# krejciadam/hammock

Measured on AMD Instinct MI355X. Metric: pairwise BLOSUM62 ShiftedScorer scores/sec (all-vs-all, thresholded neighbour list), higher is better.
Workload: dtype u8 (8-bit SWAR lanes, host-proven ranges with 16-bit / literal fallbacks; scores are int32-exact)

## Files before the change

hammock_amd/_native.py:

```python
from __future__ import annotations

import ctypes as C
import os

_HERE = os.path.dirname(os.path.abspath(__file__))
LIB_PATH = os.path.join(_HERE, "lib", "libhammock_hip.so")

HMK_OK = 0
HMK_ERR_BAD_ARG = 1
HMK_ERR_SHIFT_TOO_BIG = 2
HMK_ERR_DEVICE = 3
HMK_ERR_OOM = 4
HMK_ERR_REFERENCE_WOULD_CRASH = 5
HMK_ERR_CAPACITY = 6
HMK_ERR_NO_SEQUENCES = 7
HMK_EDGE_SHARDS = 64
HMK_MAX_LEN = 32
HMK_SURVEY_MAX_BINS = 1024
HMK_PROFILE_SYMBOLS = 21
HMK_PROFILE_MAX_WIDTH = 96
HMK_TARGET_MAX_LEN = 1 << 20
HMK_SCAN_ALL_WINDOWS = 1

SYMBOLS = [
    "hmk_abi_version", "hmk_last_kernel_ms", "hmk_create", "hmk_create_multi", "hmk_device_count", "hmk_destroy", "hmk_last_error", "hmk_set_sequences",
    "hmk_score_pairs_shifted", "hmk_score_with_shift", "hmk_score_pairs_local", "hmk_score_block_shifted", "hmk_score_block_local",
    "hmk_score_pairs_global", "hmk_score_block_global", "hmk_neighbors_global", "hmk_search_global", "hmk_align_pairs_global",
    "hmk_neighbors_shifted", "hmk_neighbors_local", "hmk_neighbors_shifted_dev", "hmk_compact_edges_dev", "hmk_pack_rows_dev", "hmk_unpack_rows_dev",
    "hmk_neighbors_last_plan", "hmk_neighbors_last_plan_shared", "hmk_neighbors_last_plan_tables", "hmk_search_shifted", "hmk_search_local", "hmk_search_best_shifted",
    "hmk_assign_shifted", "hmk_assign_local", "hmk_match_clusters_shifted", "hmk_match_clusters_local", "hmk_greedy_continue",
    "hmk_greedy_cluster", "hmk_greedy_from_edges", "hmk_greedy_from_edges_dev", "hmk_greedy_last_phases",
    "hmk_clinkage_cluster", "hmk_clinkage_from_edges", "hmk_set_java_hashset", "hmk_reserve",
    "hmk_cluster_pairs_shifted", "hmk_clinkage_merge", "hmk_clinkage_merge_from_edges",
    "hmk_cluster_linkage_shifted", "hmk_clinkage_split", "hmk_clinkage_split_from_edges",
    "hmk_components_shifted", "hmk_components_from_edges", "hmk_components_from_edges_dev",
    "hmk_cluster_align_shifted", "hmk_score_survey_shifted", "hmk_cluster_separation_shifted",
    "hmk_greedy_sweep", "hmk_greedy_sweep_from_edges", "hmk_greedy_sweep_from_edges_dev",
    "hmk_greedy_orders", "hmk_greedy_orders_from_edges",
    "hmk_representatives_shifted", "hmk_representatives_from_edges", "hmk_representatives_from_edges_dev",
    "hmk_density_shifted", "hmk_density_from_edges", "hmk_density_from_edges_dev",
    "hmk_cluster_profile", "hmk_set_targets", "hmk_scan_shifted",
]


# ... 177 lines not shown
    L.hmk_align_pairs_global.argtypes = [vp, p_u32, p_u32, u64, i32, i32, p_i32, p_u8, p_u64, p_u64]
    L.hmk_score_with_shift.argtypes = [vp, p_u32, p_u32, u64, i32, i32, p_i32, p_i32]
    L.hmk_score_block_shifted.argtypes = [vp, u32, u32, u32, u32, i32, i32, p_i32]
    L.hmk_score_block_local.argtypes = [vp, u32, u32, u32, u32, i32, i32, p_i32]
    L.hmk_score_block_global.argtypes = [vp, u32, u32, u32, u32, i32, i32, p_i32]
    L.hmk_neighbors_shifted.argtypes = [vp, i32, i32, i32, u32, u32, p_u64, u64, p_u64, C.POINTER(NeighborStats)]
    L.hmk_neighbors_local.argtypes = [vp, i32, i32, i32, u32, u32, p_u64, u64, p_u64, C.POINTER(NeighborStats)]
    L.hmk_neighbors_global.argtypes = [vp, i32, i32, i32, u32, u32, p_u64, u64, p_u64, C.POINTER(NeighborStats)]
    L.hmk_neighbors_shifted_dev.argtypes = [vp, i32, i32, i32, u32, u32, vp, u64, vp, vp]
    L.hmk_compact_edges_dev.argtypes = [vp, vp, u64, vp, vp, u64, vp, vp]
    L.hmk_pack_rows_dev.argtypes = [vp, vp, u64, vp, i32, vp, vp, u64, vp]
    L.hmk_unpack_rows_dev.argtypes = [vp, vp, vp, i32, vp, u64, vp]
    L.hmk_neighbors_last_plan.argtypes = [vp, C.POINTER(NeighborStats)]
    L.hmk_neighbors_last_plan_shared.argtypes = [vp, C.POINTER(C.c_uint32), C.POINTER(C.c_uint32)]
    L.hmk_neighbors_last_plan_tables.argtypes = [vp, C.POINTER(C.c_uint32), C.POINTER(C.c_uint64)]
    L.hmk_search_shifted.argtypes = [vp, u32, u32, u32, u32, i32, i32, i32, p_u64, u64, p_u64, C.POINTER(NeighborStats)]
    L.hmk_search_local.argtypes = [vp, u32, u32, u32, u32, i32, i32, i32, p_u64, u64, p_u64, C.POINTER(NeighborStats)]
    L.hmk_search_global.argtypes = [vp, u32, u32, u32, u32, i32, i32, i32, p_u64, u64, p_u64, C.POINTER(NeighborStats)]
    L.hmk_search_best_shifted.argtypes = [vp, u32, u32, u32, u32, i32, i32, i32, u32, p_u32, p_i32, p_u32, C.POINTER(NeighborStats)]
    L.hmk_assign_shifted.argtypes = [vp, u32, u32, u32, u32, p_u32, p_i32, u32, i32, i32, i32, u32, p_u32, p_i32, p_u32,
                                     C.POINTER(NeighborStats)]
    L.hmk_assign_local.argtypes = [vp, u32, u32, u32, u32, p_u32, p_i32, u32, i32, i32, i32, u32, p_u32, p_i32, p_u32,
                                   C.POINTER(NeighborStats)]
    L.hmk_match_clusters_shifted.argtypes = [vp, u32, u32, p_u32, u32, u32, u32, p_u32, p_i32, u32, i32, i32, i32, u32, p_u32, p_i32, p_u32,
                                             C.POINTER(NeighborStats)]
    L.hmk_match_clusters_local.argtypes = [vp, u32, u32, p_u32, u32, u32, u32, p_u32, p_i32, u32, i32, i32, i32, u32, p_u32, p_i32, p_u32,
                                           C.POINTER(NeighborStats)]
    L.hmk_greedy_continue.argtypes = [vp, u32, u32, u32, u32, p_u32, p_i32, u32, i32, i32, i32, p_i32, p_i32, C.POINTER(ContinueStats)]
    L.hmk_greedy_cluster.argtypes = [vp, i32, i32, i32, i32, p_i32, p_i32, p_i32, C.POINTER(GreedyStats)]
    L.hmk_greedy_from_edges_dev.argtypes = [vp, vp, u64, i32, i32, p_i32, p_i32, p_i32, C.POINTER(GreedyStats)]
# ... 54 lines not shown
```

hammock_amd/api.py:

```python
from __future__ import annotations

import ctypes as C

import numpy as np

from . import _native as N

AMINO_ACIDS = "ARNDCQEGHILKMFPSTWYVBZX*"
_NAME_TO_NUM = {c: i for i, c in enumerate(AMINO_ACIDS)}


class HammockException(Exception):
    """HammockException.java"""


class DataException(HammockException):
    """DataException.java -- e.g. "Shift too big" (ShiftedScorer.java:59-62)."""


class FileFormatException(HammockException):
    """FileFormatException.java"""


class DeviceError(HammockException):
# ... 544 lines not shown
            self._raise(st)

    def last_plan(self):
        stats = N.NeighborStats()
        st = N.lib.hmk_neighbors_last_plan(self._h, C.byref(stats))
        if st:
            self._raise(st)
        return stats

    def last_plan_shared(self):
        paired, shared = C.c_uint32(0), C.c_uint32(0)
        st = N.lib.hmk_neighbors_last_plan_shared(self._h, C.byref(paired), C.byref(shared))
        if st:
            self._raise(st)
        return int(paired.value), int(shared.value)

    def last_plan_tables(self):
        tiles, nbytes = C.c_uint32(0), C.c_uint64(0)
        st = N.lib.hmk_neighbors_last_plan_tables(self._h, C.byref(tiles), C.byref(nbytes))
        if st:
            self._raise(st)
        return int(tiles.value), int(nbytes.value)

    def greedy_cluster(self, max_shift, shift_penalty, threshold, max_clusters):
        cid = np.full(max(self.n, 1), -1, dtype=np.int32)
        order = np.full(max(self.n, 1), -1, dtype=np.int32)
        self.member_rank = np.zeros(max(self.n, 1), dtype=np.int32)
        stats = N.GreedyStats()
        st = N.lib.hmk_greedy_cluster(self._h, int(max_shift), int(shift_penalty), int(threshold), int(max_clusters),
                                      _ptr(cid, C.c_int32), _ptr(order, C.c_int32),
# ... 633 lines not shown
```

hammock_amd/csrc/hmk_api.cpp:

```cpp
#include "hmk_ctx.h"

using namespace hmk::impl;

extern "C" {

int hmk_abi_version(void) { return HMK_ABI_VERSION; }

double hmk_last_kernel_ms(const hmk_ctx *ctx) { return ctx ? ctx->last_kernel_ms : 0.0; }

const char *hmk_last_error(const hmk_ctx *ctx) { return ctx ? ctx->err.c_str() : g_last_error.c_str(); }

int hmk_create(const int32_t *matrix, int device, hmk_ctx **out) {
    if (!matrix || !out) return fail(nullptr, HMK_ERR_BAD_ARG, "hmk_create: null argument");
    *out = nullptr;
    hmk_ctx *ctx = new (std::nothrow) hmk_ctx();
    if (!ctx) return fail(nullptr, HMK_ERR_OOM, "out of memory");
    std::memcpy(ctx->M, matrix, sizeof(ctx->M));
    ctx->min_m = ctx->max_m = matrix[0];
    for (int e = 0; e < 576; e++) {
        ctx->min_m = std::min(ctx->min_m, matrix[e]);
        ctx->max_m = std::max(ctx->max_m, matrix[e]);
        if (matrix[e] != matrix[(e % 24) * 24 + e / 24]) ctx->symmetric = false;
        if (matrix[e] < -1000 || matrix[e] > 1000) {
            delete ctx;
// ... 253 lines not shown
    if (!ctx->plan.valid) return fail(ctx, HMK_ERR_BAD_ARG, "no neighbour pass has been planned yet");
    *stats = ctx->plan.stats;
    return HMK_OK;
}

int hmk_neighbors_last_plan_shared(hmk_ctx *ctx, uint32_t *paired_tiles, uint32_t *run_shared_tiles) {
    if (!ctx || !paired_tiles || !run_shared_tiles) return fail(ctx, HMK_ERR_BAD_ARG, "null argument");
    std::lock_guard<std::mutex> lock(ctx->mu);
    refresh_switches(ctx);
    if (!ctx->plan.valid) return fail(ctx, HMK_ERR_BAD_ARG, "no neighbour pass has been planned yet");
    *paired_tiles = ctx->plan.paired_tiles;
    *run_shared_tiles = ctx->plan.run_shared_tiles;
    return HMK_OK;
}

int hmk_neighbors_last_plan_tables(hmk_ctx *ctx, uint32_t *table_tiles, uint64_t *table_bytes) {
    if (!ctx || !table_tiles || !table_bytes) return fail(ctx, HMK_ERR_BAD_ARG, "null argument");
    std::lock_guard<std::mutex> lock(ctx->mu);
    refresh_switches(ctx);
    if (!ctx->plan.valid) return fail(ctx, HMK_ERR_BAD_ARG, "no neighbour pass has been planned yet");
    *table_tiles = ctx->plan.table_tiles;
    *table_bytes = ctx->plan.table_bytes;
    return HMK_OK;
}

int hmk_neighbors_shifted(hmk_ctx *ctx, int max_shift, int shift_penalty, int threshold, uint32_t part,
                          uint32_t n_parts, uint64_t *edges, uint64_t capacity, uint64_t *n_edges,
                          hmk_neighbor_stats *stats) {
    if (!ctx) return fail(nullptr, HMK_ERR_BAD_ARG, "null context");
    std::lock_guard<std::mutex> lock(ctx->mu);
// ... 290 lines not shown
```

hammock_amd/csrc/hmk_common.cpp:

```cpp
#include <atomic>

#include "hmk_ctx.h"
#include "hmk_grid.h"

namespace hmk {

static std::atomic<int> g_test_grid_cap{0};
void set_test_grid_cap(int cap) { g_test_grid_cap.store(cap < 1 ? 0 : cap, std::memory_order_relaxed); }
uint32_t capped_grid(const char *kernel, uint32_t wanted) {
    const int cap = g_test_grid_cap.load(std::memory_order_relaxed);
    if (cap < 1 || wanted <= (uint32_t)cap) return wanted;
    std::fprintf(stderr, "[hmk grid] %s %u -> %d\n", kernel, wanted, cap);
    return (uint32_t)cap;
}

namespace impl {

thread_local std::string g_last_error;

void Switches::read() {
    auto flag = [](const char *name) { return getenv(name) != nullptr; };
    auto num = [](const char *name, int dflt) { const char *v = getenv(name); return v ? atoi(v) : dflt; };
    *this = Switches();
    greedy_timing = flag("HMK_GREEDY_TIMING");
    no_band = flag("HMK_NO_BAND");
    no_rows_kernel = flag("HMK_NO_ROWS_KERNEL");
    key_sort = flag("HMK_NO_KEY_SORT") ? 0 : num("HMK_KEY_SORT_KEYS", 2) == 1 ? 1 : 2;
    no_row_shared = flag("HMK_NO_ROW_SHARED");
    key_row_pairs = getenv("HMK_KEY_ROW_PAIRS") ? (num("HMK_KEY_ROW_PAIRS", 0) != 0 ? 1 : 0) : -1;
    no_row_run_share = flag("HMK_NO_ROW_RUN_SHARE");
    no_tile_tables = flag("HMK_NO_TILE_TABLES");
    adj_8byte = flag("HMK_ADJ_8BYTE");
    local_literal = flag("HMK_LOCAL_LITERAL");
    local_signed = flag("HMK_LOCAL_SIGNED");
    local_no_pk = flag("HMK_LOCAL_NO_PK");
    multi_replicate = flag("HMK_MULTI_REPLICATE");
    multi_force_copies = flag("HMK_MULTI_FORCE_COPIES");
    if (const char *v = getenv("HMK_SECOND_LOOP")) second_loop = std::strcmp(v, "device") == 0 ? 1 : 2;
    phase1_threads = std::max(0, num("HMK_PHASE1_THREADS", 0));
    phase1_window = std::max(0, num("HMK_PHASE1_WINDOW", 0));
    if (const char *v = getenv("HMK_PHASE1_HOST_BAND")) {
        host_band_rows = std::max(0, atoi(v));
        if (const char *c = std::strchr(v, ',')) host_band_far_t = std::max(0, atoi(c + 1));
    }
    loop_chain = getenv("HMK_LOOP_CHAIN") ? (num("HMK_LOOP_CHAIN", 0) != 0 ? 1 : 0) : -1;
// ... 222 lines not shown
```

hammock_amd/csrc/hmk_ctx.h:

```cpp
#ifndef HMK_CTX_H
#define HMK_CTX_H
#include <hip/hip_runtime_api.h>

#include <algorithm>
#include <chrono>
#include <condition_variable>
#include <functional>
#include <future>
#include <memory>
#include <cstdio>
#include <cstdlib>
#include <cstring>
#include <map>
#include <mutex>
#include <numeric>
#include <string>
#include <tuple>
#include <thread>
#include <vector>

#include "hmk_internal.h"
#include "hmk_kernels.h"
#include "hmk_sizing.h"

// ... 68 lines not shown
    SB_SCAN_HITS, SB_SCAN_CNT,
    SB_SCAN_HASH, SB_SCAN_PAIRS, SB_SCAN_COV,
    SB_ORD_EDGES, SB_ORD_STATE, SB_ORD_POS,
    SB_ORD_IDS, SB_ORD_SUPPORT, SB_ORD_PARTNERS,
    SB_N
};

struct Switches {
    bool greedy_timing = false;
    bool no_band = false;
    bool no_rows_kernel = false;
    int key_sort = 2;
    bool no_row_shared = false;
    int key_row_pairs = -1;
    bool no_row_run_share = false;
    bool no_tile_tables = false;
    bool adj_8byte = false;
    bool local_literal = false;
    bool local_signed = false;
    bool local_no_pk = false;
    bool multi_replicate = false;
    bool multi_force_copies = false;
    int second_loop = 0;
    int phase1_threads = 0, phase1_window = 0;
    int host_band_rows = 0, host_band_far_t = 0;
    int loop_chain = -1;
    int loop_passes = 0;
    int precheck = 0;
    int late_buffers_delay_ms = 0;
    int csr_bucket_shift = 0;
// ... 16 lines not shown
struct Plan : PlanArrays {
    bool valid = false;
    int X = 0, p = 0, thr = 0;
    uint32_t part = 0, n_parts = 1;
    uint32_t band_rows = 0;
    int64_t band_req = 0;
    int lbmax = 12, lpad = 16;
    bool exact = false;
    bool rows_exact = false;
    bool no_rows_kernel = false;
    int key_sort = 2;
    bool row_shared = true;
    int key_row_pairs = -1;
    bool row_run_share = true;
    bool tile_tables = true;
    bool key_pairs = false;
    uint32_t paired_tiles = 0, run_shared_tiles = 0;
    uint32_t table_tiles = 0;
    uint64_t table_bytes = 0;
    uint32_t *d_keyrun = nullptr;
    uint32_t *d_keytab = nullptr;
    uint32_t cols_per_tile = 16384;
    uint8_t *d_mb = nullptr;
    std::vector<Group> groups;
    hmk_neighbor_stats stats{};
    uint64_t band_pairs = 0;
    uint32_t q0 = 0, q1 = 0, r0 = 0, r1 = 0;
};

struct PlanLocal : PlanArrays {
    bool valid = false;
    uint32_t part = 0, n_parts = 1;
// ... 304 lines not shown
```

hammock_amd/csrc/hmk_internal.h:

```cpp
#ifndef HMK_INTERNAL_H
#define HMK_INTERNAL_H

#include <stdint.h>

#include <functional>
#include <string>
#include <vector>

#include "../../include/hammock_hip.h"

namespace hmk {


enum { PATH_U8 = 0, PATH_U16 = 1, PATH_DIRECT = 2, PATH_ROWS = 3 };

struct TileClass {
    uint8_t la, lb;
    uint8_t nd;
    uint8_t case_b;
    uint8_t x;
    uint8_t path;
    uint8_t nw;
    uint8_t pad;
    int32_t g;
// ... 19 lines not shown
    uint64_t *edges;
    unsigned long long *counts;
    uint64_t cap_per_shard;
    uint32_t n_tiles;
    uint32_t lpad;
    uint32_t symmetric;
    uint32_t row_is_m;
    uint32_t perm_identity;
    uint32_t *deg;
    uint32_t deg_m_offset;
    const uint32_t *keyrun;
    const uint32_t *keytab;
};

constexpr int KEYTAB_DWORDS = 16;
constexpr int ROWS_KEY_PAIR_GROUPS = 2;
constexpr uint32_t ROWS_RUN_SHARED = 1u << 8;
constexpr uint32_t ROWS_TILE_TABLE = 1u << 9;
constexpr int ROWTAB_POSITIONS = 12;
constexpr int ROWTAB_DWORDS = ROWTAB_POSITIONS * 24 * 2;
constexpr int KEYGROUP_KEY_DWORDS = 2 * 24 * KEYTAB_DWORDS;
constexpr int KEYGROUP_DWORDS = KEYGROUP_KEY_DWORDS + ROWTAB_DWORDS;
constexpr bool rows_keyed(int x, int d, int cap, bool exact, int g) { return exact && d == 0 && (g == 1 || g == ROWS_KEY_PAIR_GROUPS) && x == 3 && cap == 12; }
constexpr int rows_key_pos(int x, int l, int q) { return l / 2 - 1 + q < x ? x : l / 2 - 1 + q; }

struct Nbr {
    uint32_t m;
    int32_t s;
    uint32_t id() const { return m; }
    int32_t score() const { return s; }
// ... 101 lines not shown
```

hammock_amd/csrc/hmk_plan.cpp:

```cpp
#include "hmk_ctx.h"

namespace hmk { namespace impl {

template <class T, class Cmp>
void parallel_stable_sort(std::vector<T> &v, Cmp before) {
    const size_t n = v.size();
    const unsigned hw = usable_cpus();
    size_t runs = 1;
    while (runs < 8 && runs < (hw ? hw : 1u) && n / (2 * runs) >= 32768) runs *= 2;
    if (runs == 1) { std::stable_sort(v.begin(), v.end(), before); return; }
    std::vector<size_t> cut(runs + 1);
    for (size_t r = 0; r <= runs; r++) cut[r] = n * r / runs;
    {
        std::vector<std::thread> pool;
        for (size_t r = 1; r < runs; r++) pool.emplace_back([&, r] { std::stable_sort(v.begin() + (long)cut[r], v.begin() + (long)cut[r + 1], before); });
        std::stable_sort(v.begin(), v.begin() + (long)cut[1], before);
        for (std::thread &th : pool) th.join();
    }
    std::vector<T> other(n);
    std::vector<T> *from = &v, *to = &other;
    for (size_t width = 1; width < runs; width *= 2) {
        std::vector<std::thread> pool;
        for (size_t r = 0; r < runs; r += 2 * width) {
            auto job = [&, r] {
// ... 247 lines not shown
        c.g = (int32_t)g;
        const int lpd = u16 ? 2 : 4, bits = u16 ? 16 : 8;
        const int ndw = (nd + lpd - 1) / lpd;
        c.nw = (uint8_t)ndw;
        for (int t = 0; t < nd; t++) c.cinit[t / lpd] |= (uint32_t)ci[t] << ((t % lpd) * bits);
    }
    *out = c;
}

int build_plan(hmk_ctx *ctx, int X, int p, int thr, uint32_t part, uint32_t n_parts, int64_t band_rows, bool key_sort_ok) {
    Plan &pl = ctx->plan;
    const int want_keys = key_sort_ok ? ctx->sw.key_sort : 0;
    if (pl.valid && pl.X == X && pl.p == p && pl.thr == thr && pl.part == part && pl.n_parts == n_parts &&
        (band_rows < 0 || pl.band_req == band_rows) && pl.no_rows_kernel == ctx->sw.no_rows_kernel && pl.key_sort == want_keys &&
        pl.row_shared == !ctx->sw.no_row_shared && pl.key_row_pairs == ctx->sw.key_row_pairs && pl.row_run_share == !ctx->sw.no_row_run_share &&
        pl.tile_tables == !ctx->sw.no_tile_tables)
        return HMK_OK;
    free_plan(pl);
    if (band_rows < 0) band_rows = 0;
    const int64_t band_req = band_rows;
    const bool plan_timing = ctx->sw.greedy_timing;
    const auto plan_t0 = std::chrono::steady_clock::now();
    auto plan_lap = [&](const char *what) {
        if (plan_timing)
            fprintf(stderr, "[hmk plan] %s at %.2f ms\n", what,
                    std::chrono::duration<double, std::milli>(std::chrono::steady_clock::now() - plan_t0).count());
    };
    const uint32_t n = ctx->n;
    if (n == 0) return fail(ctx, HMK_ERR_NO_SEQUENCES, "no sequences set (hmk_set_sequences)");
    if (X < 0) return fail(ctx, HMK_ERR_BAD_ARG, "max_shift must be >= 0");
    if (n_parts == 0 || part >= n_parts) return fail(ctx, HMK_ERR_BAD_ARG, "part must be < n_parts");
// ... 77 lines not shown
    if (use_rows && ctx->min_len == ctx->max_len) {
        TileClass t1;
        classify(ctx, ctx->min_len, ctx->min_len, X, p, thr, &t1);
        pl.rows_exact = (t1.path == PATH_U8 || (refine && all_rows_fit)) && rows_kernel_available(X, ctx->min_len, ctx->min_len, true);
    }
    if (!use_rows && ctx->min_len == 12 && ctx->max_len == 12 && X == 3) {
        TileClass t12;
        classify(ctx, 12, 12, X, p, thr, &t12);
        pl.exact = t12.path == PATH_U8 && t12.nw == 2;
    }
    pl.key_sort = want_keys;
    pl.row_shared = !ctx->sw.no_row_shared;
    pl.key_row_pairs = ctx->sw.key_row_pairs;
    pl.row_run_share = !ctx->sw.no_row_run_share;
    pl.tile_tables = !ctx->sw.no_tile_tables;
    std::vector<uint32_t> keyrun;
    const int L1 = ctx->min_len;
    const bool key_sorted = pl.key_sort > 0 && pl.rows_exact && !(refine && !all_rows_fit) &&
                            rows_keyed(X, 0, L1, true, rows_per_tile_rows(X, 0, L1, true) / 8) && n >= 2;
    if (key_sorted) {
        const int k0 = rows_key_pos(X, L1, 0), k1 = rows_key_pos(X, L1, 1);
        auto key_of = [&](uint32_t k) { return (uint32_t)ctx->res[ctx->off[k] + k0] * HMK_ALPHABET + ctx->res[ctx->off[k] + k1]; };
        const uint32_t b0 = band_end[L1], b1 = bucket[L1 + 1];
        std::vector<uint32_t> cnt(HMK_ALPHABET * HMK_ALPHABET + 1, 0u), sorted(perm.begin() + b0, perm.begin() + b1);
        for (uint32_t q = b0; q < b1; q++) cnt[key_of(perm[q]) + 1]++;
        for (int v = 0; v < HMK_ALPHABET * HMK_ALPHABET; v++) cnt[v + 1] += cnt[v];
        for (uint32_t q = b0; q < b1; q++) sorted[cnt[key_of(perm[q])]++] = perm[q];
        std::copy(sorted.begin(), sorted.end(), perm.begin() + b0);
        keyrun.resize(2 * (size_t)n);
        uint32_t r0 = 0, r01 = 0;
        for (uint32_t q = 0; q < n; q++) {
            const uint32_t k = perm[q], c0 = ctx->res[ctx->off[k] + k0], c1 = ctx->res[ctx->off[k] + k1];
            if (q > 0) {
                const uint32_t kp = perm[q - 1];
                const bool same0 = ctx->res[ctx->off[kp] + k0] == c0;
                r0 += same0 ? 0u : 1u;
                r01 += (pl.key_sort == 2 && same0 && ctx->res[ctx->off[kp] + k1] == c1) ? 0u : 1u;
            }
            keyrun[2 * (size_t)q] = r0 << 5 | c0;
            keyrun[2 * (size_t)q + 1] = r01 << 5 | c1;
        }
    }
    auto tiles_about = [&](uint64_t tile_rows, uint32_t cols) { return ((uint64_t)n / tile_rows / n_parts + 1) * ((uint64_t)n / (2 * cols) + 1); };
    auto cols_for = [&](uint64_t tile_rows) {
        uint32_t cols = 65536;
        while (cols > 16384 && tiles_about(tile_rows, cols) < 8 * 1792) cols /= 2;
        return cols;
    };
    constexpr uint64_t KEY_PAIR_MIN_TILES = 6 * 2048;
    const uint64_t paired_rows = key_sorted ? (uint64_t)rows_per_tile_rows(X, 0, L1, true, true) : 0;
    pl.key_pairs = paired_rows != 0 && (ctx->sw.key_row_pairs >= 0 ? ctx->sw.key_row_pairs == 1
                                                                   : tiles_about(paired_rows, cols_for(paired_rows)) >= KEY_PAIR_MIN_TILES);
    const uint64_t tile_rows = pl.key_pairs ? paired_rows : pl.rows_exact ? (uint64_t)rows_per_tile_rows(X, 0, ctx->min_len, true) : use_rows ? 16 : 6;
    pl.cols_per_tile = cols_for(tile_rows);
    while (pl.cols_per_tile > 4096 && ((uint64_t)n / tile_rows + 1) * ((uint64_t)n / (2 * pl.cols_per_tile) + 1) < 4096)
// ... 65 lines not shown
            }
            if (pl.key_pairs && pl.row_run_share && t.nrows == 8u * ROWS_KEY_PAIR_GROUPS && (t.row_shared & 3u) == 3u &&
                keys_at(t.row0 + 8) == keys_at(t.row0))
                t.row_shared |= ROWS_RUN_SHARED;
        }
        plan_lap("row-shared groups");
    }
    const bool tile_tables = key_sorted && pl.tile_tables && L1 == ROWTAB_POSITIONS;
    if (tile_tables)
        for (Tile &t : tiles) t.row_shared |= ROWS_TILE_TABLE;
    pl.table_tiles = tile_tables ? (uint32_t)tiles.size() : 0u;
    pl.table_bytes = tile_tables ? (uint64_t)((n + 7) / 8) * ROWTAB_DWORDS * 4 : 0u;
    pl.paired_tiles = pl.key_pairs ? (uint32_t)tiles.size() : 0u;
    pl.run_shared_tiles = 0;
    for (const Tile &t : tiles) pl.run_shared_tiles += (t.row_shared & ROWS_RUN_SHARED) ? 1u : 0u;

    st = upload_plan(ctx, pl, perm, (size_t)pl.lpad, 16, pl.exact ? 8 : 1, classes, tiles);
    if (!st) st = upload_biased_matrix(ctx, pl);
    if (st) return st;
    if (key_sorted) {
        if (classes.size() != 1) return fail(ctx, HMK_ERR_DEVICE, "key-sorted plan with more than one class");
        const uint32_t n_groups = (n + 7) / 8;
        const size_t tab_dwords = (size_t)n_groups * KEYGROUP_DWORDS;
        HIPCHK(ctx, hipMalloc((void **)&pl.d_keyrun, keyrun.size() * 4));
        HIPCHK(ctx, hipMemcpy(pl.d_keyrun, keyrun.data(), keyrun.size() * 4, hipMemcpyHostToDevice));
        HIPCHK(ctx, hipMalloc((void **)&pl.d_keytab, tab_dwords * 4));
        HIPCHK(ctx, launch_rows_keytab(pl.d_res_sorted, (uint32_t)pl.lpad, n, pl.d_mb, classes.at(0).case_b, X, L1, classes.at(0).cinit, pl.d_keytab,
                                       n_groups));
        if (tile_tables)
            HIPCHK(ctx, launch_rows_rowtab(pl.d_res_sorted, (uint32_t)pl.lpad, n, pl.d_mb, classes.at(0).case_b, X, L1, pl.row_shared, pl.d_keytab,
// ... 168 lines not shown
```

hammock_amd/csrc/k_neighbors_rows.h:

```cpp
#ifndef HMK_NEIGHBORS_ROWS_H
#define HMK_NEIGHBORS_ROWS_H
#include "hmk_device.h"

namespace hmk {

constexpr int ROWS_STAGE_CAPFORM = 320, ROWS_STAGE_EXACT = 640, ROWS_STAGE_SHORT = 1024;
constexpr int ROWS_INLOOP_MAXCELLS = 45;
constexpr int rows_cells(int x, int cap) { return cap * (2 * x + 1) - x * (x + 1); }
constexpr bool rows_inloop(int x, int cap) { return rows_cells(x, cap) > ROWS_INLOOP_MAXCELLS; }
constexpr bool rows_inloop_shape(int x, int d, int cap, bool exact) { return (exact && d > 0) || rows_inloop(x, cap); }
constexpr int rows_stage(int x, int d, int cap, bool exact) {
    return !exact ? ROWS_STAGE_CAPFORM : rows_inloop_shape(x, d, cap, exact) ? ROWS_STAGE_EXACT : ROWS_STAGE_SHORT;
}
constexpr int rows_groups(int x, int , int cap, bool exact) {
    return !exact ? 2 : rows_inloop(x, cap) ? 1 : 2;
}
constexpr bool rows_two_ended(int x, int d, int cap, bool exact, int g) { return exact && !rows_inloop_shape(x, d, cap, exact) && g == 2; }

template <typename T>
__device__ __forceinline__ T rows_table_read(uint32_t addr) {
    return *reinterpret_cast<const volatile HMK_LDS T *>((uintptr_t)addr);
}
constexpr int rows_waves(int nd, int cap, int lds_bytes, bool exact) {
    const int v = cap + 2 * nd + 36 + (exact ? 0 : 6);
// ... 188 lines not shown
            n += 2 * ((ops + 1) / 2) + ((role == 1 || role == 2) && halves == 2 ? 1 : 0);
        }
        return n;
    }
    static constexpr bool follower_covers(int skip) {
        if (!body_covers(skip, true)) return false;
        for (int u = 0; u < ND; u++)
            for (int j = plane_j0(u); j < plane_j1(u); j++) {
                int n = (ordinary(u, skip, true, j) ? 1 : 0) + (skipped(skip, j) ? 1 : 0);
                for (int h = 0; h < 2; h++)
                    if (run_carried(u, skip) && merged_half(u, skip, true, h) && merged_j(u, h) == j) n += (j + u - X == key_pos(h)) ? 1 : 2;
                if (n != 1) return false;
            }
        return true;
    }

    template <int GI, int SKIP = 0, bool RS = false>
    static __device__ __forceinline__ void accumulate(const uint32_t (&off)[CAP], const uint32_t (&toff)[NT], int lbs,
                                                      const uint32_t (&c0)[ND], const uint32_t (&c1)[ND], uint32_t (&W0)[ND], uint32_t (&W1)[ND]) {
        static_assert(SKIP == 0 || EXACT_LB, "key positions are skipped by the one-length forms only");
        static_assert(!RS || EXACT_LB, "row-shared groups: one-length forms only");
        const uint32_t (&ci)[ND] = c0;
        if constexpr (RS) {
            static_assert(body_covers(SKIP, true), "every cell of the overlap exactly once");
            u32x2 ml = {0u, 0u}, mh = {0u, 0u};
#pragma unroll
            for (int u = 0; u < ND; u++) {
                const bool hi = merged_half(u, SKIP, true, 1), lo = merged_half(u, SKIP, true, 0);
                if (hi) {
                    if (merged_reuse(u, SKIP, true)) mh = ml;
// ... 440 lines not shown

    const uint8_t *const res_sorted = P.res_sorted;
    const uint32_t lpad_s = P.lpad;

    constexpr bool INLOOP = rows_inloop_shape(X, D, CAP, EXACT_LB);
    constexpr bool DEFER = EXACT_LB && !INLOOP;
    const uint64_t ka64 = (uint64_t)(uintptr_t)__builtin_amdgcn_kernarg_segment_ptr();
    const uint32_t ka_lo = (uint32_t)ka64, ka_hi = (uint32_t)(ka64 >> 32);
    uint32_t acc[G];
#pragma unroll
    for (int g = 0; g < G; g++) acc[g] = 0;
    static_assert(!KEYED || (G <= 2 && 2 * ND <= KEYTAB_DWORDS), "key table entry; at most two row groups per tile");
    static_assert(!KEYED || (S::body_reads(3, false) == 58 && S::body_reads(1, false) == 65 && S::body_reads(0, false) == 72), "ordinary bodies");
    static_assert(!KEYED || (S::body_reads(3, true) == 54 && S::body_reads(1, true) == 60 && S::body_reads(0, true) == 66), "row-shared bodies (and the lead of a run-shared tile)");
    static_assert(!KEYED || (S::follower_reads(3) == 48 && S::follower_reads(1) == 53 && S::follower_reads(0) == 58), "followers of a run-shared tile");
    static_assert(!KEYED || (S::run_carried_planes(3) == 6 && S::run_carried_planes(1) == 7 && S::run_carried_planes(0) == 7), "dwords a lead hands over");
    static_assert(!KEYED || (S::run_body_adds(3, 2) == 62 && S::run_body_adds(1, 2) == 69 && S::run_body_adds(0, 2) == 75 && S::run_body_adds(3, 3) == 58 &&
                             S::run_body_adds(1, 3) == 64 && S::run_body_adds(0, 3) == 68), "sums of the lead and the follower");
    const uint32_t wave = __builtin_amdgcn_readfirstlane(tid >> 6);
    const uint32_t *kt_tile = nullptr, *kr_wave = nullptr;
    if (keyed) {
        kt_tile = P.keytab + (size_t)(T.row0 >> 3) * KEYGROUP_DWORDS;
        kr_wave = P.keyrun + 2 * (size_t)(T.col0 + wave * 64);
    }
    auto key_entry = [](const uint32_t *e, uint32_t (&k0)[ND], uint32_t (&k1)[ND]) {
#pragma unroll
        for (int u = 0; u + 1 < ND; u += 2) {
            const u32x4 a = rows_const_load<u32x4>(e + 2 * u);
            k0[u] = a.x; k1[u] = a.y; k0[u + 1] = a.z; k1[u + 1] = a.w;
        }
        if constexpr (ND & 1) {
            const u32x2 a = rows_const_load<u32x2>(e + 2 * (ND - 1));
            k0[ND - 1] = a.x; k1[ND - 1] = a.y;
        }
    };
    using No = std::false_type;
    using Yes = std::true_type;
    constexpr bool RUNS = KEYED && G >= 2;
    for (uint32_t bt = 0; bt < n_batches; bt++) {
        const uint32_t colrel = bt * 256 + tid;
        const uint32_t col = T.col0 + colrel;
        uint32_t words[S::LPADW], tw[S::TWN];
        S::load_words(res_sorted + (size_t)col * lpad_s, col < col_end, RUNS && interior, lbs, words, tw);
        int kmode = 0;
        u32x2 ra;
        if constexpr (KEYED) {
            const uint32_t wc0 = T.col0 + bt * 256 + wave * 64;
            if (keyed && wc0 < col_end) {
                const uint32_t last = min(63u, col_end - 1u - wc0);
                ra = rows_const_load<u32x2>(kr_wave);
                const u32x2 rb = rows_const_load<u32x2>(kr_wave + 2 * last);
                if (ra.x == rb.x) kmode = ra.y == rb.y ? 3 : 1;
            }
        }
        uint32_t off[CAP], toff[S::NT];
        S::offsets_of(words, tw, tab_addr, tab_addr, off, toff);
        const bool look = !DEFER || (bt & 3u) == 3u || bt + 1 == n_batches;
        uint32_t Pm[ND];

        if constexpr (RUNS) {
            static_assert(INLOOP && !DEFER && !TWO, "paired tiles: an in-loop shape");
            auto body = [&](auto gt, auto kt, auto rt, uint32_t (&W0)[ND], uint32_t (&W1)[ND]) __attribute__((always_inline)) {
                constexpr int g = decltype(gt)::value, KM = decltype(kt)::value;
                constexpr bool RUN = decltype(rt)::value;
                const uint32_t *const kt_group = kt_tile + (size_t)g * KEYGROUP_DWORDS;
                [[maybe_unused]] const bool row_shared = (rs_groups & (1u << g)) != 0;
                uint32_t ks0[ND], ks1[ND];
                if constexpr (KM == 3) {
                    uint32_t kb0[ND], kb1[ND];
                    key_entry(kt_group + (ra.x & 31u) * KEYTAB_DWORDS, ks0, ks1);
                    key_entry(kt_group + (24 + (ra.y & 31u)) * KEYTAB_DWORDS, kb0, kb1);
#pragma unroll
                    for (int u = 0; u < ND; u++) { ks0[u] += kb0[u]; ks1[u] += kb1[u]; }
                } else if constexpr (KM == 1) {
                    key_entry(kt_group + (ra.x & 31u) * KEYTAB_DWORDS, ks0, ks1);
#pragma unroll
                    for (int u = 0; u < ND; u++) asm volatile("" : "+s"(ks0[u]), "+s"(ks1[u]));
                }
                const uint32_t (&s0)[ND] = KM != 0 ? ks0 : ci;
                const uint32_t (&s1)[ND] = KM != 0 ? ks1 : ci;
                read_phase_begin(prio);
                if constexpr (RUN) S::template accumulate_run<g, KM, (g > 0)>(off, s0, s1, W0, W1, Pm);
                else if (row_shared) S::template accumulate<g, KM, true>(off, toff, lbs, s0, s1, W0, W1);
                else S::template accumulate<g, KM>(off, toff, lbs, s0, s1, W0, W1);
                read_phase_end(prio);
            };
            auto hits = [&](auto gt, auto ft, const uint32_t (&W0)[ND], const uint32_t (&W1)[ND]) __attribute__((always_inline)) {
                constexpr int g = decltype(gt)::value;
                constexpr bool FULL = decltype(ft)::value;
                uint32_t o0 = W0[0], o1 = W1[0];
#pragma unroll
                for (int u = 1; u < ND; u++) { o0 |= W0[u]; o1 |= W1[u]; }
                if (__ballot(((o0 | o1) & 0x80808080u) != 0) == 0) return;
                uint32_t rm0 = 0x80808080u, rm1 = 0x80808080u;
                if constexpr (!FULL) {
                    const uint32_t rows_here = T.nrows - 8 * g;
                    rm0 = rows_here >= 4 ? 0x80808080u : 0x80808080u & ((1u << (8 * rows_here)) - 1u);
                    rm1 = rows_here >= 8 ? 0x80808080u : rows_here <= 4 ? 0u : 0x80808080u & ((1u << (8 * (rows_here - 4))) - 1u);
                }
                uint32_t hm = ((o0 & rm0) >> 4) | (o1 & rm1);
// ... 144 lines not shown
                                else stage[cnt + mbcnt64(mask)] = rec;
                            }
                            hm &= hm - 1u;
                        }
                        if constexpr (TWO && g == 1) cnt_hi += (uint32_t)__popcll(mask);
                        else cnt += (uint32_t)__popcll(mask);
                    }
                    if (!full) break;
                    flush_stage_rows<X, D, CAP, EXACT_LB, G, MODE>(stage, cnt, cnt_hi, tab_addr, ka_lo, ka_hi);
                    cnt = 0;
                    cnt_hi = 0;
                }
            };
            rows_for_each_group(std::make_integer_sequence<int, G>{}, one_group);
        }
        kr_wave += 2 * 256;
    }
    flush_stage_rows<X, D, CAP, EXACT_LB, G, MODE>(stage, cnt, cnt_hi, tab_addr, ka_lo, ka_hi);
}

template <int X, int D, int CAP, bool EXACT_LB, int G, int MODE>
__global__ void __launch_bounds__(256, rows_waves(2 * X + D + 1, CAP, rows_lds_bytes(X, D, CAP, EXACT_LB, G), EXACT_LB))
k_neighbors_rows(const NeighborParams P, const uint32_t tile_base) {
    __shared__ __attribute__((aligned(16))) uint8_t smem[rows_lds_bytes(X, D, CAP, EXACT_LB, G)];
    rows_tile<X, D, CAP, EXACT_LB, G, MODE>(P, tile_base, smem);
}

constexpr int ROWS_LENS_MAXLA = 20;
constexpr int rows_lens_first(int capb) { return capb <= 12 ? 6 : capb <= 16 ? 13 : 17; }
constexpr bool rows_lens_has(int x, int d, int capb, int lb) { return lb >= rows_lens_first(capb) && lb <= capb && lb >= 2 * x && lb + d <= ROWS_LENS_MAXLA; }
constexpr int rows_lens_lds(int x, int d, int capb) {
// ... 35 lines not shown
```

include/hammock_hip.h:

```cpp
#ifndef HAMMOCK_HIP_H
#define HAMMOCK_HIP_H

#include <stdint.h>

#ifdef __cplusplus
extern "C" {
#endif

#define HMK_ABI_VERSION 4
#define HMK_ALPHABET 24
#define HMK_MAX_LEN 32
#define HMK_MAX_SEQUENCES (1u << 24)
#define HMK_EDGE_SHARDS 64

typedef enum {
    HMK_OK = 0,
    HMK_ERR_BAD_ARG = 1,
    HMK_ERR_SHIFT_TOO_BIG = 2,
    HMK_ERR_DEVICE = 3,
    HMK_ERR_OOM = 4,
    HMK_ERR_REFERENCE_WOULD_CRASH = 5,
    HMK_ERR_CAPACITY = 6,
    HMK_ERR_NO_SEQUENCES = 7
} hmk_status;
// ... 58 lines not shown
int hmk_neighbors_global(hmk_ctx *ctx, int gap_open, int gap_extend, int threshold, uint32_t part,
                         uint32_t n_parts, uint64_t *edges, uint64_t capacity, uint64_t *n_edges,
                         hmk_neighbor_stats *stats);

int hmk_neighbors_shifted_dev(hmk_ctx *ctx, int max_shift, int shift_penalty, int threshold,
                              uint32_t part, uint32_t n_parts, void *d_edges, uint64_t capacity,
                              void *d_counts, void *stream);
int hmk_compact_edges_dev(hmk_ctx *ctx, const void *d_edges, uint64_t capacity, const void *d_counts,
                          void *d_out, uint64_t out_capacity, void *d_total, void *stream);
int hmk_pack_rows_dev(hmk_ctx *ctx, const void *d_edges, uint64_t capacity, const void *d_counts, int threshold,
                      void *d_row_start, void *d_adj, uint64_t adj_capacity, void *stream);
int hmk_unpack_rows_dev(hmk_ctx *ctx, const void *d_row_start, const void *d_adj, int threshold, void *d_edges_out,
                        uint64_t out_capacity, void *stream);
int hmk_neighbors_last_plan(hmk_ctx *ctx, hmk_neighbor_stats *stats);
int hmk_neighbors_last_plan_shared(hmk_ctx *ctx, uint32_t *paired_tiles, uint32_t *run_shared_tiles);
int hmk_neighbors_last_plan_tables(hmk_ctx *ctx, uint32_t *table_tiles, uint64_t *table_bytes);


int hmk_search_shifted(hmk_ctx *ctx, uint32_t q0, uint32_t q1, uint32_t r0, uint32_t r1,
                       int max_shift, int shift_penalty, int threshold,
                       uint64_t *edges, uint64_t capacity, uint64_t *n_edges, hmk_neighbor_stats *stats);
int hmk_search_local(hmk_ctx *ctx, uint32_t q0, uint32_t q1, uint32_t r0, uint32_t r1,
                     int gap_open, int gap_extend, int threshold,
                     uint64_t *edges, uint64_t capacity, uint64_t *n_edges, hmk_neighbor_stats *stats);
int hmk_search_global(hmk_ctx *ctx, uint32_t q0, uint32_t q1, uint32_t r0, uint32_t r1,
                      int gap_open, int gap_extend, int threshold,
                      uint64_t *edges, uint64_t capacity, uint64_t *n_edges, hmk_neighbor_stats *stats);
int hmk_search_best_shifted(hmk_ctx *ctx, uint32_t q0, uint32_t q1, uint32_t r0, uint32_t r1,
                            int max_shift, int shift_penalty, int threshold, uint32_t k,
                            uint32_t *hit_index, int32_t *hit_score, uint32_t *n_hits,
// ... 442 lines not shown
```

Baseline: 2664 billion.

## Keep key-skipping fast path for windows straddling one key-run boundary

Widens the per-column key-run record to four dwords so it also stores where the column's two-key run starts. A 64-column wave window that crosses exactly one boundary between key runs now takes the both-keys-skipped path. Lanes past the boundary then add a scalar-loaded correction, the difference between two key-table entries, to their accumulators. Before, such windows fell back to the slower single-key or no-key path. The cost is twice the key-run memory and extra scalar loads and adds on split windows. Plan statistics and an env switch to disable the feature are also added.

```diff
diff --git a/hammock_amd/_native.py b/hammock_amd/_native.py
--- a/hammock_amd/_native.py
+++ b/hammock_amd/_native.py
@@ -27,7 +27,7 @@
     "hmk_score_pairs_shifted", "hmk_score_with_shift", "hmk_score_pairs_local", "hmk_score_block_shifted", "hmk_score_block_local",
     "hmk_score_pairs_global", "hmk_score_block_global", "hmk_neighbors_global", "hmk_search_global", "hmk_align_pairs_global",
     "hmk_neighbors_shifted", "hmk_neighbors_local", "hmk_neighbors_shifted_dev", "hmk_compact_edges_dev", "hmk_pack_rows_dev", "hmk_unpack_rows_dev",
-    "hmk_neighbors_last_plan", "hmk_neighbors_last_plan_shared", "hmk_neighbors_last_plan_tables", "hmk_search_shifted", "hmk_search_local", "hmk_search_best_shifted",
+    "hmk_neighbors_last_plan", "hmk_neighbors_last_plan_shared", "hmk_neighbors_last_plan_split", "hmk_neighbors_last_plan_tables", "hmk_search_shifted", "hmk_search_local", "hmk_search_best_shifted",
     "hmk_assign_shifted", "hmk_assign_local", "hmk_match_clusters_shifted", "hmk_match_clusters_local", "hmk_greedy_continue",
     "hmk_greedy_cluster", "hmk_greedy_from_edges", "hmk_greedy_from_edges_dev", "hmk_greedy_last_phases",
     "hmk_clinkage_cluster", "hmk_clinkage_from_edges", "hmk_set_java_hashset", "hmk_reserve",
@@ -235,6 +235,7 @@
     L.hmk_neighbors_last_plan.argtypes = [vp, C.POINTER(NeighborStats)]
     L.hmk_neighbors_last_plan_shared.argtypes = [vp, C.POINTER(C.c_uint32), C.POINTER(C.c_uint32)]
     L.hmk_neighbors_last_plan_tables.argtypes = [vp, C.POINTER(C.c_uint32), C.POINTER(C.c_uint64)]
+    L.hmk_neighbors_last_plan_split.argtypes = [vp, C.POINTER(C.c_uint64), C.POINTER(C.c_uint64), C.POINTER(C.c_uint64)]
     L.hmk_search_shifted.argtypes = [vp, u32, u32, u32, u32, i32, i32, i32, p_u64, u64, p_u64, C.POINTER(NeighborStats)]
     L.hmk_search_local.argtypes = [vp, u32, u32, u32, u32, i32, i32, i32, p_u64, u64, p_u64, C.POINTER(NeighborStats)]
     L.hmk_search_global.argtypes = [vp, u32, u32, u32, u32, i32, i32, i32, p_u64, u64, p_u64, C.POINTER(NeighborStats)]
diff --git a/hammock_amd/api.py b/hammock_amd/api.py
--- a/hammock_amd/api.py
+++ b/hammock_amd/api.py
@@ -582,6 +582,13 @@
         if st:
             self._raise(st)
         return int(paired.value), int(shared.value)
+
+    def last_plan_split(self):
+        w, s, k = C.c_uint64(0), C.c_uint64(0), C.c_uint64(0)
+        st = N.lib.hmk_neighbors_last_plan_split(self._h, C.byref(w), C.byref(s), C.byref(k))
+        if st:
+            self._raise(st)
+        return int(w.value), int(s.value), int(k.value)
 
     def last_plan_tables(self):
         tiles, nbytes = C.c_uint32(0), C.c_uint64(0)
diff --git a/hammock_amd/csrc/hmk_api.cpp b/hammock_amd/csrc/hmk_api.cpp
--- a/hammock_amd/csrc/hmk_api.cpp
+++ b/hammock_amd/csrc/hmk_api.cpp
@@ -291,6 +291,17 @@
     return HMK_OK;
 }
 
+int hmk_neighbors_last_plan_split(hmk_ctx *ctx, uint64_t *windows, uint64_t *straddling_windows, uint64_t *split_windows) {
+    if (!ctx || !windows || !straddling_windows || !split_windows) return fail(ctx, HMK_ERR_BAD_ARG, "null argument");
+    std::lock_guard<std::mutex> lock(ctx->mu);
+    refresh_switches(ctx);
+    if (!ctx->plan.valid) return fail(ctx, HMK_ERR_BAD_ARG, "no neighbour pass has been planned yet");
+    *windows = ctx->plan.key_windows;
+    *straddling_windows = ctx->plan.straddling_windows;
+    *split_windows = ctx->plan.split_windows;
+    return HMK_OK;
+}
+
 int hmk_neighbors_last_plan_tables(hmk_ctx *ctx, uint32_t *table_tiles, uint64_t *table_bytes) {
     if (!ctx || !table_tiles || !table_bytes) return fail(ctx, HMK_ERR_BAD_ARG, "null argument");
     std::lock_guard<std::mutex> lock(ctx->mu);
diff --git a/hammock_amd/csrc/hmk_common.cpp b/hammock_amd/csrc/hmk_common.cpp
--- a/hammock_amd/csrc/hmk_common.cpp
+++ b/hammock_amd/csrc/hmk_common.cpp
@@ -29,6 +29,7 @@
     no_row_shared = flag("HMK_NO_ROW_SHARED");
     key_row_pairs = getenv("HMK_KEY_ROW_PAIRS") ? (num("HMK_KEY_ROW_PAIRS", 0) != 0 ? 1 : 0) : -1;
     no_row_run_share = flag("HMK_NO_ROW_RUN_SHARE");
+    no_key_split = flag("HMK_NO_KEY_SPLIT");
     no_tile_tables = flag("HMK_NO_TILE_TABLES");
     adj_8byte = flag("HMK_ADJ_8BYTE");
     local_literal = flag("HMK_LOCAL_LITERAL");
diff --git a/hammock_amd/csrc/hmk_ctx.h b/hammock_amd/csrc/hmk_ctx.h
--- a/hammock_amd/csrc/hmk_ctx.h
+++ b/hammock_amd/csrc/hmk_ctx.h
@@ -106,6 +106,7 @@
     bool no_row_shared = false;
     int key_row_pairs = -1;
     bool no_row_run_share = false;
+    bool no_key_split = false;
     bool no_tile_tables = false;
     bool adj_8byte = false;
     bool local_literal = false;
@@ -152,8 +153,10 @@
     int key_row_pairs = -1;
     bool row_run_share = true;
     bool tile_tables = true;
+    bool key_split = true;
     bool key_pairs = false;
     uint32_t paired_tiles = 0, run_shared_tiles = 0;
+    uint64_t key_windows = 0, straddling_windows = 0, split_windows = 0;
     uint32_t table_tiles = 0;
     uint64_t table_bytes = 0;
     uint32_t *d_keyrun = nullptr;
diff --git a/hammock_amd/csrc/hmk_internal.h b/hammock_amd/csrc/hmk_internal.h
--- a/hammock_amd/csrc/hmk_internal.h
+++ b/hammock_amd/csrc/hmk_internal.h
@@ -57,6 +57,7 @@
 };
 
 constexpr int KEYTAB_DWORDS = 16;
+constexpr int KEYRUN_DWORDS = 4;
 constexpr int ROWS_KEY_PAIR_GROUPS = 2;
 constexpr uint32_t ROWS_RUN_SHARED = 1u << 8;
 constexpr uint32_t ROWS_TILE_TABLE = 1u << 9;
diff --git a/hammock_amd/csrc/hmk_plan.cpp b/hammock_amd/csrc/hmk_plan.cpp
--- a/hammock_amd/csrc/hmk_plan.cpp
+++ b/hammock_amd/csrc/hmk_plan.cpp
@@ -285,7 +285,7 @@
     if (pl.valid && pl.X == X && pl.p == p && pl.thr == thr && pl.part == part && pl.n_parts == n_parts &&
         (band_rows < 0 || pl.band_req == band_rows) && pl.no_rows_kernel == ctx->sw.no_rows_kernel && pl.key_sort == want_keys &&
         pl.row_shared == !ctx->sw.no_row_shared && pl.key_row_pairs == ctx->sw.key_row_pairs && pl.row_run_share == !ctx->sw.no_row_run_share &&
-        pl.tile_tables == !ctx->sw.no_tile_tables)
+        pl.tile_tables == !ctx->sw.no_tile_tables && pl.key_split == !ctx->sw.no_key_split)
         return HMK_OK;
     free_plan(pl);
     if (band_rows < 0) band_rows = 0;
@@ -393,6 +393,7 @@
     pl.key_row_pairs = ctx->sw.key_row_pairs;
     pl.row_run_share = !ctx->sw.no_row_run_share;
     pl.tile_tables = !ctx->sw.no_tile_tables;
+    pl.key_split = !ctx->sw.no_key_split;
     std::vector<uint32_t> keyrun;
     const int L1 = ctx->min_len;
     const bool key_sorted = pl.key_sort > 0 && pl.rows_exact && !(refine && !all_rows_fit) &&
@@ -406,18 +407,21 @@
         for (int v = 0; v < HMK_ALPHABET * HMK_ALPHABET; v++) cnt[v + 1] += cnt[v];
         for (uint32_t q = b0; q < b1; q++) sorted[cnt[key_of(perm[q])]++] = perm[q];
         std::copy(sorted.begin(), sorted.end(), perm.begin() + b0);
-        keyrun.resize(2 * (size_t)n);
-        uint32_t r0 = 0, r01 = 0;
+        keyrun.assign((size_t)KEYRUN_DWORDS * n, 0u);
+        uint32_t r0 = 0, r01 = 0, start = 0;
         for (uint32_t q = 0; q < n; q++) {
             const uint32_t k = perm[q], c0 = ctx->res[ctx->off[k] + k0], c1 = ctx->res[ctx->off[k] + k1];
             if (q > 0) {
                 const uint32_t kp = perm[q - 1];
                 const bool same0 = ctx->res[ctx->off[kp] + k0] == c0;
                 r0 += same0 ? 0u : 1u;
-                r01 += (pl.key_sort == 2 && same0 && ctx->res[ctx->off[kp] + k1] == c1) ? 0u : 1u;
+                const bool same01 = pl.key_sort == 2 && same0 && ctx->res[ctx->off[kp] + k1] == c1;
+                r01 += same01 ? 0u : 1u;
+                if (!same01) start = q;
             }
-            keyrun[2 * (size_t)q] = r0 << 5 | c0;
-            keyrun[2 * (size_t)q + 1] = r01 << 5 | c1;
+            keyrun[(size_t)KEYRUN_DWORDS * q] = r0 << 5 | c0;
+            keyrun[(size_t)KEYRUN_DWORDS * q + 1] = r01 << 5 | c1;
+            keyrun[(size_t)KEYRUN_DWORDS * q + 2] = start;
         }
     }
     auto tiles_about = [&](uint64_t tile_rows, uint32_t cols) { return ((uint64_t)n / tile_rows / n_parts + 1) * ((uint64_t)n / (2 * cols) + 1); };
@@ -513,6 +517,22 @@
     pl.paired_tiles = pl.key_pairs ? (uint32_t)tiles.size() : 0u;
     pl.run_shared_tiles = 0;
     for (const Tile &t : tiles) pl.run_shared_tiles += (t.row_shared & ROWS_RUN_SHARED) ? 1u : 0u;
+    pl.key_windows = pl.straddling_windows = pl.split_windows = 0;
+    const bool splits = key_sorted && pl.key_pairs && pl.key_sort == 2 && pl.key_split;
+    if (key_sorted && !splits)
+        for (uint32_t q = 0; q < n; q++) keyrun[(size_t)KEYRUN_DWORDS * q + 2] = 0u;
+    if (key_sorted && pl.key_pairs) {
+        for (const Tile &t : tiles)
+            for (uint32_t w0 = t.col0; w0 < t.col0 + t.ncols; w0 += 64) {
+                const uint32_t last = std::min(63u, t.col0 + t.ncols - 1u - w0);
+                const uint32_t *a = &keyrun[(size_t)KEYRUN_DWORDS * w0], *b = &keyrun[(size_t)KEYRUN_DWORDS * (w0 + last)];
+                pl.key_windows++;
+                if (a[1] == b[1]) continue;
+                pl.straddling_windows++;
+                if ((b[1] >> 5) - (a[1] >> 5) == 1u && b[2] - w0 - 1u < last) pl.split_windows++;
+            }
+        plan_lap("split windows");
+    }
 
     st = upload_plan(ctx, pl, perm, (size_t)pl.lpad, 16, pl.exact ? 8 : 1, classes, tiles);
     if (!st) st = upload_biased_matrix(ctx, pl);
diff --git a/hammock_amd/csrc/k_neighbors_rows.h b/hammock_amd/csrc/k_neighbors_rows.h
--- a/hammock_amd/csrc/k_neighbors_rows.h
+++ b/hammock_amd/csrc/k_neighbors_rows.h
@@ -226,6 +226,16 @@
             }
         return true;
     }
+    static constexpr int split_starts(int side, int which) { return (which == 0 ? 1 : 0) + (side == 1 ? (which == 1 ? 1 : -1) : 0); }
+    static constexpr bool split_covers(bool rs) {
+        for (int side = 0; side < 2; side++)
+            if (split_starts(side, side) != 1 || split_starts(side, 1 - side) != 0) return false;
+        for (int u = 0; u < ND; u++)
+            for (int j = plane_j0(u); j < plane_j1(u); j++)
+                if (skipped(3, j) != (j == key_pos(0) || j == key_pos(1))) return false;
+        return rs ? follower_covers(3) : body_covers(3, false);
+    }
+    static constexpr int split_adds() { return 2 * ND; }
 
     template <int GI, int SKIP = 0, bool RS = false>
     static __device__ __forceinline__ void accumulate(const uint32_t (&off)[CAP], const uint32_t (&toff)[NT], int lbs,
@@ -696,14 +706,15 @@
     static_assert(!KEYED || (S::body_reads(3, false) == 58 && S::body_reads(1, false) == 65 && S::body_reads(0, false) == 72), "ordinary bodies");
     static_assert(!KEYED || (S::body_reads(3, true) == 54 && S::body_reads(1, true) == 60 && S::body_reads(0, true) == 66), "row-shared bodies (and the lead of a run-shared tile)");
     static_assert(!KEYED || (S::follower_reads(3) == 48 && S::follower_reads(1) == 53 && S::follower_reads(0) == 58), "followers of a run-shared tile");
-    static_assert(!KEYED || (S::run_carried_planes(3) == 6 && S::run_carried_planes(1) == 7 && S::run_carried_planes(0) == 7), "dwords a lead hands over");
+    static_assert(!KEYED || (S::body_reads(3, false) == 58 && S::body_reads(3, true) == 54 && S::follower_reads(3) == 48), "a split window reads what a both-keys window reads");
+    static_assert(!KEYED || (S::run_carried_planes(3) == 6&& S::run_carried_planes(1) == 7 && S::run_carried_planes(0) == 7), "dwords a lead hands over");
     static_assert(!KEYED || (S::run_body_adds(3, 2) == 62 && S::run_body_adds(1, 2) == 69 && S::run_body_adds(0, 2) == 75 && S::run_body_adds(3, 3) == 58 &&
                              S::run_body_adds(1, 3) == 64 && S::run_body_adds(0, 3) == 68), "sums of the lead and the follower");
     const uint32_t wave = __builtin_amdgcn_readfirstlane(tid >> 6);
     const uint32_t *kt_tile = nullptr, *kr_wave = nullptr;
     if (keyed) {
         kt_tile = P.keytab + (size_t)(T.row0 >> 3) * KEYGROUP_DWORDS;
-        kr_wave = P.keyrun + 2 * (size_t)(T.col0 + wave * 64);
+        kr_wave = P.keyrun + KEYRUN_DWORDS * (size_t)(T.col0 + wave * 64);
     }
     auto key_entry = [](const uint32_t *e, uint32_t (&k0)[ND], uint32_t (&k1)[ND]) {
 #pragma unroll
@@ -726,13 +737,21 @@
         S::load_words(res_sorted + (size_t)col * lpad_s, col < col_end, RUNS && interior, lbs, words, tw);
         int kmode = 0;
         u32x2 ra;
+        [[maybe_unused]] uint32_t split = 0;
         if constexpr (KEYED) {
             const uint32_t wc0 = T.col0 + bt * 256 + wave * 64;
             if (keyed && wc0 < col_end) {
                 const uint32_t last = min(63u, col_end - 1u - wc0);
                 ra = rows_const_load<u32x2>(kr_wave);
-                const u32x2 rb = rows_const_load<u32x2>(kr_wave + 2 * last);
-                if (ra.x == rb.x) kmode = ra.y == rb.y ? 3 : 1;
+                if constexpr (KEYED && G >= 2) {
+                    const u32x4 rb = rows_const_load<u32x4>(kr_wave + KEYRUN_DWORDS * last);
+                    const bool two = (rb.y >> 5) - (ra.y >> 5) == 1u && rb.z - wc0 - 1u < last;
+                    split = two ? (rb.z - T.col0) | (rb.x & 31u) << 16 | (rb.y & 31u) << 21 : 0u;
+                    kmode = ra.y == rb.y || two ? 3 : ra.x == rb.x ? 1 : 0;
+                } else {
+                    const u32x2 rb = rows_const_load<u32x2>(kr_wave + KEYRUN_DWORDS * last);
+                    if (ra.x == rb.x) kmode = ra.y == rb.y ? 3 : 1;
+                }
             }
         }
         uint32_t off[CAP], toff[S::NT];
@@ -749,6 +768,7 @@
                 [[maybe_unused]] const bool row_shared = (rs_groups & (1u << g)) != 0;
                 uint32_t ks0[ND], ks1[ND];
                 if constexpr (KM == 3) {
+                    static_assert(S::split_covers(false) && S::split_covers(true), "a split window adds every cell of the overlap exactly once");
                     uint32_t kb0[ND], kb1[ND];
                     key_entry(kt_group + (ra.x & 31u) * KEYTAB_DWORDS, ks0, ks1);
                     key_entry(kt_group + (24 + (ra.y & 31u)) * KEYTAB_DWORDS, kb0, kb1);
@@ -766,6 +786,39 @@
                 else if (row_shared) S::template accumulate<g, KM, true>(off, toff, lbs, s0, s1, W0, W1);
                 else S::template accumulate<g, KM>(off, toff, lbs, s0, s1, W0, W1);
                 read_phase_end(prio);
+                if constexpr (KM == 3) {
+                    static_assert(S::split_adds() == 14, "a split window's correction: one add per accumulator dword");
+                    if (split != 0) {
+                        uint32_t sp = split, rx = ra.x, ry = ra.y;
+                        asm volatile("" : "+s"(sp), "+s"(rx), "+s"(ry));
+                        const uint32_t start = sp & 0xFFFFu, c0 = (sp >> 16) & 31u, c1 = sp >> 21;
+                        auto correct = [&](const uint32_t *first, const uint32_t *second) __attribute__((always_inline)) {
+                            uint64_t fa = (uint64_t)(uintptr_t)first, sa = (uint64_t)(uintptr_t)second;
+                            if (colrel >= start) {
+                                rows_static_for<(ND + 1) / 2>([&](auto ht) __attribute__((always_inline)) {
+                                    constexpr int U = 2 * decltype(ht)::value;
+                                    asm volatile("" : "+s"(fa), "+s"(sa));
+                                    const uint32_t *f = (const uint32_t *)(uintptr_t)fa, *e = (const uint32_t *)(uintptr_t)sa;
+                                    if constexpr (U + 1 < ND) {
+                                        const u32x4 a = rows_const_load<u32x4>(f + 2 * U), b = rows_const_load<u32x4>(e + 2 * U);
+                                        uint32_t d0 = b.x - a.x, d1 = b.y - a.y, d2 = b.z - a.z, d3 = b.w - a.w;
+                                        asm volatile("" : "+s"(d0), "+s"(d1), "+s"(d2), "+s"(d3));
+                                        W0[U] += d0; W1[U] += d1; W0[U + 1] += d2; W1[U + 1] += d3;
+                                        asm volatile("" : "+v"(W0[U]), "+v"(W1[U]), "+v"(W0[U + 1]), "+v"(W1[U + 1]), "+s"(fa), "+s"(sa));
+                                    } else {
+                                        const u32x2 a = rows_const_load<u32x2>(f + 2 * U), b = rows_const_load<u32x2>(e + 2 * U);
+                                        uint32_t d0 = b.x - a.x, d1 = b.y - a.y;
+                                        asm volatile("" : "+s"(d0), "+s"(d1));
+                                        W0[U] += d0; W1[U] += d1;
+                                        asm volatile("" : "+v"(W0[U]), "+v"(W1[U]));
+                                    }
+                                });
+                            }
+                        };
+                        correct(kt_group + (24 + (ry & 31u)) * KEYTAB_DWORDS, kt_group + (24 + c1) * KEYTAB_DWORDS);
+                        if ((rx & 31u) != c0) correct(kt_group + (rx & 31u) * KEYTAB_DWORDS, kt_group + c0 * KEYTAB_DWORDS);
+                    }
+                }
             };
             auto hits = [&](auto gt, auto ft, const uint32_t (&W0)[ND], const uint32_t (&W1)[ND]) __attribute__((always_inline)) {
                 constexpr int g = decltype(gt)::value;
@@ -940,7 +993,7 @@
             };
             rows_for_each_group(std::make_integer_sequence<int, G>{}, one_group);
         }
-        kr_wave += 2 * 256;
+        kr_wave += KEYRUN_DWORDS * 256;
     }
     flush_stage_rows<X, D, CAP, EXACT_LB, G, MODE>(stage, cnt, cnt_hi, tab_addr, ka_lo, ka_hi);
 }
diff --git a/include/hammock_hip.h b/include/hammock_hip.h
--- a/include/hammock_hip.h
+++ b/include/hammock_hip.h
@@ -96,6 +96,7 @@
                         uint64_t out_capacity, void *stream);
 int hmk_neighbors_last_plan(hmk_ctx *ctx, hmk_neighbor_stats *stats);
 int hmk_neighbors_last_plan_shared(hmk_ctx *ctx, uint32_t *paired_tiles, uint32_t *run_shared_tiles);
+int hmk_neighbors_last_plan_split(hmk_ctx *ctx, uint64_t *windows, uint64_t *straddling_windows, uint64_t *split_windows);
 int hmk_neighbors_last_plan_tables(hmk_ctx *ctx, uint32_t *table_tiles, uint64_t *table_bytes);
 
 
```

Result: slower. 2536 billion (-4.8%).
